# Xinglab/abPOA

Measured on AMD Instinct MI355X. Metric: read-sets/sec (consensus bit-exact) + DP Gcells/sec (roofline.dp_gcells_per_s), higher is better.
Workload: dtype int16

## Files before the change

### abpoa_amd/csrc/engine_options.cpp

```cpp
#include "engine_options.h"
#include <atomic>
#include <cstdlib>
#include <cstring>
#include <mutex>
#include <string>

namespace abpoa_hip {
namespace {

struct Row { const char *name, *help; };
const Row kTable[] = {
    {"ABPOA_GPU_DEVICES", "P  device ordinals abpoa_hip_msa_batch spreads its batches over: all | 0,1,... (default: the device of abpoa_hip_init)"},
    {"ABPOA_GPU_BATCHES_PER_DEVICE", "P  batches dealt per device queue [2]"},
    {"ABPOA_HIP_STRICT", "P  1: a call that would hand any read-set to the host driver fails with ABPOA_HIP_ESTRICT"},
    {"ABPOA_HIP_VERBOSE", "P  per-pass timings, residency and fallback reasons on stderr"},
    {"ABPOA_HIP_HOSTGRAPH", "T  1: the host driver for every job"},
    {"ABPOA_HIP_NO_DEVICE_STRAND", "T  1: -s jobs on the host driver"},
    {"ABPOA_HIP_NO_DEVICE_LOCAL", "T  1: local-mode jobs on the host driver"},
    {"ABPOA_HIP_NO_DEVICE_GENERAL", "T  1: general-kernel jobs on the host driver"},
    {"ABPOA_HIP_DEVICE_GENERAL", "T  1: the general kernel for every device-resident job"},
    {"ABPOA_HIP_LOCKSTEP", "T  1: one launch per phase and round also where the all-rounds kernel would run"},
    {"ABPOA_HIP_NODIR", "T  1: score-record arenas instead of direction words"},
    {"ABPOA_HIP_DIR_WIDE", "T  1 / 0: direction words for wide-band alignments always / never (default: by residency and memory)"},
    {"ABPOA_HIP_NOFAST", "T  1: no fast row loops (general kernel)"},
    {"ABPOA_HIP_NOWIDE", "T  1: no wide row loop"},
    {"ABPOA_HIP_NOXL", "T  1: no long-read form of the wide row loop"},
    {"ABPOA_HIP_TEAM", "T  1 | 2 | 4 wavefronts per wide-band alignment"},
    {"ABPOA_HIP_LOCAL_TEAM", "T  1 / 0: the four-wavefront local row loop always / never"},
    {"ABPOA_HIP_WIDE_LO", "T  smallest band half-width that takes the wide loop [40]"},
    {"ABPOA_HIP_RING_ROWS", "T  depth of the wide loop's score ring (4 | 8 | 16)"},
    {"ABPOA_HIP_EXTRA_ROUTE_MIN", "T  ragged sets with fewer extra columns keep the narrow loop"},
    {"ABPOA_HIP_NO_RAGGED_SPLIT", "T  1: read-sets with ragged read ends stay in the batch of the uniform ones (no all-rounds kernel for such a job)"},
    {"ABPOA_HIP_RAGGED_CONCURRENT", "T  1: the ragged batch of a mixed job runs on a second queue of the device beside the uniform batch (measured: see LOG.md)"},
    {"ABPOA_HIP_PASS_SETS", "T  read-sets per pass of the device-resident driver"},
    {"ABPOA_HIP_FIRST_PASS", "T  start the node-slot ladder at pass 1 / 2 / 3 (profiling runs of one step)"},
    {"ABPOA_HIP_NO_PASS_HINT", "T  1: always start the ladder at 3x"},
    {"ABPOA_HIP_GROUPS", "T  read-set groups of the host driver"},
    {"ABPOA_HIP_ARENA_PCT", "T  arena estimate in percent (overflow-retry tests)"},
    {"ABPOA_HIP_BT_BYTES", "T  LDS window of the tail kernel in bytes"},
    {"ABPOA_HIP_BT_WC", "T  columns per row of the tail's column-slice windows"},
    {"ABPOA_HIP_ORDER_LDS", "T  0: the row-order walk with global tables"},
    {"ABPOA_HIP_ORDER_CAP", "T  node capacity of the row-order walk's LDS tables"},
    {"ABPOA_HIP_DBG", "D  bit mask handed to the kernels (DevBatch.dbg: 64 no fast loops, 128 keep counters, 1024 one wavefront per backtrack, 2048 the compiler's tight loop, ...)"},
    {"ABPOA_HIP_DEVSYNC", "D  1: compare device graph / row order / MSA with the host's after every read"},
    {"ABPOA_HIP_DEVICE_AUDIT", "D  1: every pool of a device queue must sit on that queue's device"},
    {"ABPOA_HIP_CIGAR_DIGEST", "D  1: fold every graph cigar into a per-set digest on the device"},
    {"ABPOA_HIP_DIRTRACE", "D  1: keep direction words and scores (word-level tests)"},
    {"ABPOA_HIP_IMBAL", "D  1: per-round mean / slowest alignment"},
    {"ABPOA_HIP_WIDE_COUNTERS", "D  path census of the wide loop (diagnostic build)"},
    {"ABPOA_HIP_ROW_CENSUS", "D  row census of the narrow loop (diagnostic build)"},
    {"ABPOA_HIP_ORDER_PROF", "D  in-kernel clock of the row-order walk (diagnostic build)"},
};
constexpr int N = (int)(sizeof(kTable) / sizeof(kTable[0]));

struct Snap { bool set[N]; std::string val[N]; };
std::mutex g_mu;
bool g_over_on[N]; std::string g_over[N];
std::atomic<const Snap *> g_snap{nullptr};

int find(const char *name) { for (int i = 0; i < N; ++i) if (strcmp(kTable[i].name, name) == 0) return i; return -1; }

}

void refresh_options() {
    std::lock_guard<std::mutex> lk(g_mu);
    Snap s;
    for (int i = 0; i < N; ++i) {
        const char *e = g_over_on[i] ? g_over[i].c_str() : getenv(kTable[i].name);
        s.set[i] = e != nullptr; s.val[i] = e ? e : "";
    }
    const Snap *cur = g_snap.load(std::memory_order_acquire);
    bool same = cur != nullptr;
    for (int i = 0; same && i < N; ++i) same = cur->set[i] == s.set[i] && cur->val[i] == s.val[i];
    if (!same) g_snap.store(new Snap(s), std::memory_order_release);
}

// ... 22 lines not shown
```

### abpoa_amd/csrc/rows_fast.h

```cpp
#pragma once
#include "dp_common.h"
#include "dir_plane.h"
#include "rows_tight_asm.h"
#include "wide_closed_forms.h"

namespace abpoa_hip {

template <typename T, int GAP> struct FastFmt { static constexpr int CW = GAP == 0 ? 2 : (GAP == 1 ? 4 : 8); };
template <typename T, int GAP> struct DirFmt {
    static constexpr int DB = GAP == 1 ? 2 : 4;
    static constexpr int UPV2 = Width<T>::PN * DB / 16;
    __device__ __host__ static constexpr int units(int nv) { return (nv * UPV2 + 1) >> 1; }
};
template <int GAP> __device__ __forceinline__ unsigned dir_word(unsigned kf, unsigned u1, unsigned u2, unsigned d1, unsigned d2) {
    static_assert(DIRA_DF1_SH - DIRA_UE1_SH == 3 && DIRC_UE2_SH - DIRC_UE1_SH == 3 && DIRC_DF2_SH - DIRC_DF1_SH == 3 && DIRC_DF1_SH - DIRC_UE1_SH == 8, "field layout of dir_plane.h");
    if (GAP == 1) return (((d1 << 3) | u1) << DIRA_UE1_SH) | kf;
    return (((((d2 << 3) | d1) << 8) | ((u2 << 3) | u1)) << DIRC_UE1_SH) | kf;
}
template <int GAP> __device__ __forceinline__ unsigned dir_pack(unsigned kM, unsigned kE1, unsigned kE2, unsigned u1, unsigned u2, unsigned d1, unsigned d2) {
    return dir_word<GAP>(GAP == 1 ? (kE1 << DIRA_KE1_SH) | kM : (((kE2 << 4) | kE1) << DIRC_KE1_SH) | kM, u1, u2, d1, d2);
}
__device__ __forceinline__ unsigned umin_(unsigned a, unsigned b) { return a < b ? a : b; }
template <typename T> __device__ __forceinline__ unsigned dir_literal(int Hm1, int Fm1, int F, int oe, int e) {
    return (int)(T)(Hm1 - oe) == F ? (unsigned)DIR_LIT_OPEN : ((int)(T)(Fm1 - e) == F ? (unsigned)DIR_LIT_EXT : (unsigned)DIR_LIT_NEITHER);
// ... 100 lines not shown
    typedef __attribute__((address_space(3))) int lds_int_t;
    const int vslot = (int)(unsigned)(size_t)(lds_int_t *)fr + 4 * ((threadIdx.x & 63 & (RR - 1)) * (NPW * RCS) + 2);
    auto ring_at = [&](int slot_addr, int col_idx) __attribute__((always_inline)) { return (const int *)(lds_int_t *)(size_t)(unsigned)(slot_addr + 4 * col_idx); };
    int *s_mx = (int *)(lds_raw + (WPLAN ? b.lds.w_mx_off : b.lds.mx_off));
    auto qat = [&](int j) __attribute__((always_inline)) -> int {
        if constexpr (WPLAN) return ((int)s_query[j >> 1] >> ((j & 1) * 4)) & 15; else return (int)s_query[j];
    };
    const int infw = I16 ? (int)(((unsigned)inf & 0xffffu) | ((unsigned)inf << 16)) : inf;
    const int qlen_sn = qlen / PN;
    auto wr = [](int x) __attribute__((always_inline)) { return (int)(T)x; };

    const int idist = inj_dist<PN>(l);
    const int inj1 = idist >= 0 ? inf - idist * e1 : INT_MIN, inj2 = idist >= 0 ? inf - idist * e2 : INT_MIN;
    const int le1 = lane * e1, le2 = lane * e2;
    const int cf1 = oe1 - e1 + le1, cf2 = oe2 - e2 + le2;
    const long long lo_ll = (long long)(I16 ? INT16_MIN : INT32_MIN) + imax(oe1, oe2) + (long long)PN * imax(e1, e2);
    const int fast_lo = (int)lo_ll;
    const int kconst = I16 ? argmax_key16_const(PN, l, vvl) : 0;
    const int ktie = argmax_tie32(PN, l, vvl);

    { GLOBAL_AS const int32_t *g_mat = vgpr_ptr(b.mat); for (int i = tid; i < m * m1; i += NT) { const int bb = i / m1, qc = i - bb * m1; s_mx[i] = qc < m ? g_mat[bb * m + qc] : 0; } }
    for (int i = tid; i < RR * NPW * RCS; i += NT) { const int pl = (i / RCS) % NPW; fr[i] = (I16 && pl == 0) ? infw : ((EPACK && pl == 1) ? 0 : inf); }
    if (NW > 1 && tid < 16) xch[tid] = make_int4(INT_MIN, INT_MIN, I16 ? 0 : INT_MIN, 0);
    WG_SYNC();
    auto ring_put = [&](int slot, int x, int H, int E1, int E2) __attribute__((always_inline)) {
        int *q = fr + slot * (NPW * RCS) + 2 + x;
        if (I16) { q[0] = (int)(((unsigned)H & 0xffffu) | ((unsigned)E1 << 16)); if (GAP == 2) q[RCS] = E2; }
        else { q[0] = H; if (GAP != 0) q[RCS] = E1; if (GAP == 2) q[2 * RCS] = E2; }
    };

    const bool extend = sgpr(b.align_mode == ABPOA_HIP_EXTEND_MODE ? 1 : 0) != 0;
    int ex_best = inf, ex_i = 0, ex_j = 0, ex_rem = 0; bool zstop = false;
    const bool asm_tight_on = sgpr(!(b.dbg & 2048) && RC == 128 && b.align_mode != ABPOA_HIP_EXTEND_MODE ? 1 : 0) != 0;
    int cur = 0, n_vec_lane = 0;
    const int cap_pn = (int)(d.plane_cap / PN > 0x7fffffffLL ? 0x7fffffffLL : d.plane_cap / PN);
    const int cap_turbo = cap_pn - (DIR ? dir_units(NV) + NV * CWR : NV * CW);
    const int remain_end = __builtin_amdgcn_readfirstlane(io.row_remain[gn - 1]);
    int vg_geo = 0, vg_mi = 0, vg_off = 0;
    int vg_vm = 0, rowmax = 0;
    {
        const int r = __builtin_amdgcn_readfirstlane(io.row_remain[0]) - remain_end - 1;
        const int dp_end0 = imin(qlen, imax(0, qlen - r) + w);
        const int end_sn0 = dp_end0 / PN, W0 = (end_sn0 + 1) * PN;
        if ((long long)W0 * CWR > d.plane_cap) { status = ABPOA_HIP_STATUS_OVERFLOW; cursor_out = 0; n_cells_out = 0; rows_done_out = 0; return; }
        const bool ring0 = W0 <= RC && !EPACK;
        T *H = io.planes;
        for (int i = tid; i < W0; i += NT) {
            int h, x1 = inf, x2 = inf, f1 = inf, f2 = inf;
            if (GAP == 0) h = wr(-e1 * i);
            else if (GAP == 1) { const int g = wr(-o1 - e1 * i); h = i == 0 ? 0 : g; x1 = i == 0 ? wr(-oe1) : inf; f1 = i == 0 ? inf : g; }
            else {
                const int g1 = wr(-o1 - e1 * i), g2 = wr(-o2 - e2 * i);
                h = i == 0 ? 0 : imax(g1, g2); x1 = i == 0 ? wr(-oe1) : inf; x2 = i == 0 ? wr(-oe2) : inf; f1 = i == 0 ? inf : g1; f2 = i == 0 ? inf : g2;
            }
            T *cellp = H + (long long)i * CWR;
            if constexpr (CPK) { cellp[0] = (T)h; cellp[1] = (T)(i == 0 ? (int)((unsigned)(h - x1) | ((unsigned)(h - x2) << 16)) : -1); }
            else if constexpr (CSP) { cellp[0] = (T)h; cellp[PL_E1] = (T)x1; if (GAP == 2) { cellp[PL_E2] = (T)x2; cellp[3] = (T)0; } }
            else if constexpr (GAP == 0) { cellp[0] = (T)h; cellp[1] = (T)0; }
            else {
                cellp[0] = (T)h; cellp[PL_E1] = (T)x1; cellp[PL_F1] = (T)f1;
                if (GAP == 2) { cellp[PL_E2] = (T)x2; cellp[PL_F2] = (T)f2; }
            }
            if (ring0) ring_put(0, i, h, x1, x2);
        }
        cur = (end_sn0 + 1) * CWR;
        if (lane == 0) { vg_geo = (end_sn0 << 12) | (ring0 ? GEO_RING : 0); vg_mi = 0; vg_off = DIR ? cur : 0; }
// ... 12 lines not shown
    auto load_b = [&](const MetaA &a) __attribute__((always_inline)) {
        MetaB q; const int np = a.pe - a.ps;
#pragma unroll
        for (int k = 0; k < NPM; ++k) q.p[k] = io.pred_row[a.ps + imin(k, imax(np - 1, 0))];
        return q;
    };
    MetaA a1 = load_a(0); MetaB b1 = load_b(a1); MetaA a2 = load_a(64);
    int tv_r1 = 0, tv_r2 = 0;
    int tv_meta = 0, tv_rterm = 0, tv_ps = 0, tv_p0 = 0, tv_p1 = 0, tv_p2 = 0, tv_p3 = 0;
    int tv_p4 = 0, tv_p5 = 0, tv_p6 = 0, tv_p7 = 0;
    int tv_tb = 0;
    auto switch_tile = [&](int t0) __attribute__((always_inline)) {
        const int myrow = t0 + lane, np = a1.pe - a1.ps;
        bool fastrow = np >= 1 && np <= 4 && myrow < gn - 1 && myrow >= 1;
#pragma unroll
        for (int k = 0; k < 4; ++k) { const int dk = myrow - b1.p[k]; fastrow = fastrow && dk >= 1 && dk < RR; }
        tv_meta = (a1.base & 0xff) | (imin(np, 255) << 8) | (fastrow ? (1 << 16) : 0);
        if (!WPLAN) {
            tv_meta |= ((fastrow && np <= 2 && RC <= 128) ? (1 << 17) : 0) | ((fastrow && np >= 3 && RC <= 128) ? (1 << 18) : 0);
            bool row8 = np >= 5 && np <= 8 && myrow < gn - 1 && myrow >= 1 && RC <= 128;
#pragma unroll
            for (int k = 0; k < NPM; ++k) { const int dk = myrow - b1.p[k]; row8 = row8 && dk >= 1 && dk < RR; }
            tv_meta |= row8 ? (1 << 20) : 0;
        }
        {
            bool widerow = np >= 1 && np <= 8 && myrow < gn - 1 && myrow >= 1;
#pragma unroll
            for (int k = 0; k < NPM; ++k) { const int dk = myrow - b1.p[k]; widerow = widerow && dk >= 1 && dk < ((WIDEB || !WPLAN) ? 64 : RR); }
            tv_meta |= widerow ? (1 << 19) : 0;
        }
        if constexpr (DIR) {
            const bool sp = a1.sd >= RR;
            if (sp) { tv_meta |= 1 << 21; if (tv_meta & (1 << 17)) tv_meta = (tv_meta & ~(1 << 17)) | (1 << 22); }
        }
        tv_tb = ((myrow - b1.p[0]) & 0xff) | (((myrow - b1.p[1]) & 0xff) << 8) | (((a1.base & 0xff) * m1 * 4) << 16);
        tv_rterm = qlen - (a1.rem - remain_end - 1); tv_ps = a1.ps;
        tv_r1 = imin(gn, tv_rterm) - w; tv_r2 = tv_rterm + w;
        tv_p0 = b1.p[0]; tv_p1 = b1.p[1]; tv_p2 = b1.p[2]; tv_p3 = b1.p[3];
        tv_p4 = b1.p[4]; tv_p5 = b1.p[5]; tv_p6 = b1.p[6]; tv_p7 = b1.p[7];
        a1 = a2; b1 = load_b(a1); a2 = load_a(t0 + 128);
    };
    int qc_beg_sn = -1, qoff0 = 0, qoff1 = 0;
    auto geo_of = [&](int p, int row, int &geo, int &mi, int &off) __attribute__((always_inline)) {
        if (row - p < 64) { const int sl = p & 63; geo = __builtin_amdgcn_readlane(vg_geo, sl); mi = __builtin_amdgcn_readlane(vg_mi, sl); off = __builtin_amdgcn_readlane(vg_off, sl); }
        else {
            geo = __builtin_amdgcn_readfirstlane(gld_i32(io.g_bsn + p) | (gld_i32(io.g_esn + p) << 12)); mi = __builtin_amdgcn_readfirstlane(gld_i32(io.row_max_i + p));
            off = __builtin_amdgcn_readfirstlane((int)(uint32_t)(gld_i64(io.g_coff + p) / PN));
        }
    };
    int beg_sn = 0, end_sn = 0, off_pn = 0, max_pe = 0, rterm = 0, base = 0, np = 0;
    bool to_ring = false;
    unsigned am_key = 0; int am_val = INT_MIN, am_v = 0, am_isend = 0; bool am_any = false;

    auto set_band = [&](auto pin, int mn_mi, int mx_mi, int min_pb) __attribute__((always_inline)) {
        auto S = [](int x) __attribute__((always_inline)) { if constexpr (decltype(pin)::value) return sgpr(x); else return x; };
        const int left = S(imin(gn, mn_mi + 1)), right = S(decltype(pin)::value ? mx_mi + 1 : imax(0, mx_mi + 1));
        const int lo = S(imin(left, rterm) - w), hi = S(imax(right, rterm) + w);
        const int beg = S(imax(0, lo)), end = S(imin(qlen, hi));
        beg_sn = imax((int)((unsigned)beg / PN), min_pb); end_sn = (int)((unsigned)end / PN);
    };
    auto refresh_qc = [&]() __attribute__((always_inline)) {
        if (beg_sn != qc_beg_sn) {
            qc_beg_sn = beg_sn;
            const int c0 = beg_sn * PN + lane, c1 = c0 + 64;
            qoff0 = (c0 >= 1 && c0 <= qlen) ? qat(c0 - 1) : m; qoff1 = (c1 >= 1 && c1 <= qlen) ? qat(c1 - 1) : m;
        }
// ... 932 lines not shown
                            }
                        }
                    }
                    if (lane == 0) { bcast[0] = rc; bcast[1] = beg_sn; bcast[2] = end_sn; bcast[3] = off_pn; bcast[4] = mi; bcast[5] = to_ring ? 1 : 0; bcast[6] = cur; bcast[7] = rowmax; }
                }
                lds_barrier();
                rc = __builtin_amdgcn_readfirstlane(bcast[0]); beg_sn = __builtin_amdgcn_readfirstlane(bcast[1]); end_sn = __builtin_amdgcn_readfirstlane(bcast[2]);
                off_pn = __builtin_amdgcn_readfirstlane(bcast[3]); mi = __builtin_amdgcn_readfirstlane(bcast[4]); to_ring = __builtin_amdgcn_readfirstlane(bcast[5]) != 0;
                cur = __builtin_amdgcn_readfirstlane(bcast[6]); rowmax = __builtin_amdgcn_readfirstlane(bcast[7]);
                if (rc == 2) { status = ABPOA_HIP_STATUS_OVERFLOW; break; }
                commit_row(ti, to_ring);
                lds_barrier();
                ++row;
                continue;
            }
            int ok_ = 1;
            if constexpr (!WPLAN && GAP != 0) if (__builtin_expect(two_chunk_streak, 0)) {
                const int ti_ = row & 63, meta_ = __builtin_amdgcn_readlane(tv_meta, ti_);
                if constexpr (DIR) row_spill = (meta_ >> 21) & 1;
                if ((meta_ >> 19) & 1) {
                    CENSUS_T0()
                    last_done = row;
                    rterm = __builtin_amdgcn_readlane(tv_rterm, ti_); base = meta_ & 0xff; np = (meta_ >> 8) & 0xff;
                    const int nch_ = ilp_band(row, ti_);
                    if (nch_ == -2) { status = ABPOA_HIP_STATUS_OVERFLOW; break; }
                    if (nch_ == 2 && ilp_chunks(std::integral_constant<int, 2>{}, nch_, row, ti_) == 1) { commit_row(ti_, true); CENSUS(3) ++row; continue; }
                }
                two_chunk_streak = 0;
            }
            bool cxx_tight = true;
#if !defined(ABPOA_HIP_ABLATE) && !defined(ABPOA_HIP_PROFILE) && (!defined(ABPOA_HIP_ROW_CENSUS) || defined(ABPOA_HIP_ASM_CENSUS)) && !defined(ABPOA_HIP_NO_ASM_TIGHT)
            if constexpr (!WPLAN && I16 && GAP == 1 && DIR) {
                if (asm_tight_on && cur + NV * (r_hi - row) <= cap_turbo) {
                    int code, sM, sTB, sRT, sR2, sP0, sM0, sG0, sSL0, sA, sB, sESN, sBSN, sPB0, sPE0, sNV1, sC0, sP1, sM1, sG1, sSL1, sPB1, sPE1, sP2, sSL2, sPB2, sPE2, sP3, sSL3, sPB3, sPE3;
                    long long inb, amok, msk;
#ifdef ABPOA_HIP_ASM_CENSUS
                    const int asm_row0 = row; const long long asm_t0 = (long long)__builtin_amdgcn_s_memtime();
#endif
                    int infw_v = infw, inf_v = inf; asm("" : "+v"(infw_v), "+v"(inf_v));
                    const int mxb = (int)(unsigned)(size_t)(lds_int_t *)s_mx, qb = (int)(unsigned)(size_t)(lds_int_t *)(const void *)s_query;
                    asm volatile(TIGHT_ASM_I16_AFFINE_DIR
                        : [row] "+s"(row), [cur] "+s"(cur), [qcb] "+s"(qc_beg_sn), [code] "=&s"(code), [geo] "+v"(vg_geo), [mi] "+v"(vg_mi), [off] "+v"(vg_off), [qoff0] "+v"(qoff0),
                          [qoff1] "+v"(qoff1), [sM] "=&s"(sM), [sTB] "=&s"(sTB), [sRT] "=&s"(sRT), [sR2] "=&s"(sR2), [sP0] "=&s"(sP0), [sM0] "=&s"(sM0), [sG0] "=&s"(sG0), [sSL0] "=&s"(sSL0), [sA] "=&s"(sA),
                          [sB] "=&s"(sB), [sESN] "=&s"(sESN), [sBSN] "=&s"(sBSN), [sPB0] "=&s"(sPB0), [sPE0] "=&s"(sPE0), [sNV1] "=&s"(sNV1), [sC0] "=&s"(sC0), [sP1] "=&s"(sP1),
                          [sM1] "=&s"(sM1), [sG1] "=&s"(sG1), [sSL1] "=&s"(sSL1), [sPB1] "=&s"(sPB1), [sPE1] "=&s"(sPE1), [sP2] "=&s"(sP2), [sSL2] "=&s"(sSL2), [sPB2] "=&s"(sPB2),
                          [sPE2] "=&s"(sPE2), [sP3] "=&s"(sP3), [sSL3] "=&s"(sSL3), [sPB3] "=&s"(sPB3), [sPE3] "=&s"(sPE3), [inb] "=&s"(inb), [amok] "=&s"(amok), [msk] "=&s"(msk)
                        : [lane] "v"(lane), [tvmeta] "v"(tv_meta), [tvtb] "v"(tv_tb), [tvr1] "v"(tv_r1), [tvr2] "v"(tv_r2), [tvp2] "v"(tv_p2), [tvp3] "v"(tv_p3), [vslot] "v"(vslot), [le1] "v"(le1), [cf1] "v"(cf1), [inj1] "v"(inj1), [kN] "v"(kN),
                          [kE] "v"(kE), [vvl] "v"(vvl), [vl] "v"(l), [infwv] "v"(infw_v), [infv] "v"(inf_v), [c1] "s"(1 - w), [c2] "s"(1 + w), [qlen] "s"(qlen), [rc] "s"(RC), [mxb] "s"(mxb), [fastlo] "s"(fast_lo),
                          [e1] "s"(e1), [oe1] "s"(oe1), [infk] "s"((int)((((unsigned)(inf + 32768)) << 16) | 0xffffu)), [planes] "s"(io.planes), [rhi] "s"(r_hi), [qb] "s"(qb), [m] "s"(m), [perm] "s"(0x05040100)
                        : "v92", "v93", "v94", "v95", "v96", "v97", "v98", "v99", "v100", "v101", "v102", "v103", "v104", "v105", "v106", "v107", "v108", "v109", "v110", "v111", "v112", "v113", "v114", "v115", "v116", "v117", "v118", "v119",
                          "v120", "v121", "v122", "v123", "v124", "v125", "v126", "v127", "vcc", "scc", "m0", "memory");
                    ok_ = code == 1 ? 0 : (code == 2 ? -1 : 1);
                    cxx_tight = false;
#ifdef ABPOA_HIP_ASM_CENSUS
                    fseg[0] += ((long long)(row - asm_row0) << 40) + ((long long)__builtin_amdgcn_s_memtime() - asm_t0);
#endif
                }
            }
#endif
            if constexpr (!WPLAN) if (cxx_tight) for (;;) {
                const int ti_ = row & 63;
                const int meta_ = __builtin_amdgcn_readlane(tv_meta, ti_);
                if (!__builtin_expect((meta_ >> 17) & 1, 1)) break;
                if constexpr (DIR) row_spill = (meta_ >> 21) & 1;
                CENSUS_T0()
                rterm = __builtin_amdgcn_readlane(tv_rterm, ti_);
                base = meta_ & 0xff; np = (meta_ >> 8) & 0xff;
                ok_ = np == 1 ? turbo_body(std::integral_constant<int, 1>{}, std::false_type{}, row, ti_) : turbo_body(std::integral_constant<int, 2>{}, std::false_type{}, row, ti_);
                if (__builtin_expect(ok_ != 1, 0)) break;
                commit_row(ti_, true);
                CENSUS(np == 1 ? 0 : 1)
                if (++row >= r_hi || zstop) break;
            }
            last_done = row - 1;
            if (row >= r_hi || zstop) break;
            const int ti = row & 63;
            last_done = row;
            CENSUS_T0()
            const int meta = __builtin_amdgcn_readlane(tv_meta, ti);
            rterm = __builtin_amdgcn_readlane(tv_rterm, ti);
// ... 134 lines not shown
```

### abpoa_amd/csrc/rows_tight_asm.h

```cpp
#pragma once
#define TA_SDWA0 " dst_sel:DWORD dst_unused:UNUSED_PAD src0_sel:WORD_0 src1_sel:DWORD\n\t"
#define TA_SDWA_S1W0 " dst_sel:DWORD dst_unused:UNUSED_PAD src0_sel:DWORD src1_sel:WORD_0\n\t"
#define TA_SDWA_S1W1 " dst_sel:DWORD dst_unused:UNUSED_PAD src0_sel:DWORD src1_sel:WORD_1\n\t"
#define TA_SDWA_S0W1 " dst_sel:DWORD dst_unused:UNUSED_PAD src0_sel:WORD_1 src1_sel:DWORD\n\t"
#define TA_DPP(CTRL) " " CTRL " bank_mask:0xf\n\t"
#define vQA "v104"
#define vCOL "v105"
#define vX "v106"
#define vQ "v107"
#define vR0 "v108"
#define vR1 "v109"
#define vR01 "v[108:109]"
#define vKC "v110"
#define vH "v111"
#define vHSE "v112"
#define vAK "v113"
#define vS1 "v114"
#define vG "v115"
#define vF "v115"
#define vQD "v116"
#define vRO "v117"
#define vHO "v118"
#define vT2A "v119"
#define vEN "v120"
// ... 130 lines not shown
    S("v_lshl_or_b32 " vWD ", " vSH ", 14, " vWD "\n\t")                                                     \
    "global_store_short " vRO ", " vWD ", %[planes]\n\t"                                                     \
    "v_cndmask_b32_e64 " vHE ", %[infwv], " vHE ", %[inb]\n\t"                                                   \
    "ds_write2st64_b32 " vQD ", " vHE ", %[infwv] offset1:1\n\t"                                             \
    "v_readlane_b32 %[sA], " vAK ", 63\n\t"                                                                  \
    "s_bitset1_b32 %[sB], 24\n\t"                                                                            \
    "v_writelane_b32 %[geo], %[sB], m0\n\t"     "v_writelane_b32 %[off], %[cur], m0\n\t"                     \
    "s_and_b32 %[sM0], %[sA], 63\n\t"           "s_add_i32 %[sM0], %[sM0], %[sC0]\n\t"                       \
    "s_cmp_gt_u32 %[sA], %[infk]\n\t"           "s_cselect_b32 %[sA], %[sM0], -1\n\t"       \
    "v_writelane_b32 %[mi], %[sA], m0\n\t"                                                                   \
    "s_add_i32 %[cur], %[cur], %[sNV1]\n\t"     "s_add_i32 %[cur], %[cur], 1\n\t"                            \
    "s_add_i32 %[row], %[row], 1\n\t"           "s_cmp_lt_i32 %[row], %[rhi]\n\t"     "s_cbranch_scc1 L_row_%=\n\t"

#define TA_IF4_YES(x) x
#define TA_IF4_NO(x) ""
#define TA_FOLD(LANE, SL, PB, PE)                                                                            \
    "v_readlane_b32 %[sM1], %[mi], " LANE "\n\t"  "v_readlane_b32 %[sG1], %[geo], " LANE "\n\t"  "v_readlane_b32 " SL ", %[vslot], " LANE "\n\t" \
    "s_min_i32 %[sA], %[sA], %[sM1]\n\t"          "s_max_i32 %[sB], %[sB], %[sM1]\n\t"           "s_and_b32 %[sG0], %[sG0], %[sG1]\n\t" \
    "s_and_b32 " PB ", %[sG1], 0xfff\n\t"         "s_bfe_u32 " PE ", %[sG1], 0xc000c\n\t"
#define TA_READK(X, PAIR, SL, PB, PE)                                                                        \
    "s_lshl_b32 %[sA], " PB ", 4\n\t"             "v_subrev_u32 " X ", %[sA], " vCOL "\n\t"                  \
    "v_add_u32 " vT ", -1, " X "\n\t"             "v_med3_i32 " vT ", " vT ", -2, %[rc]\n\t"                 \
    "v_lshl_add_u32 " vT ", " vT ", 2, " SL "\n\t"  "ds_read2_b32 " PAIR ", " vT " offset1:1\n\t"            \
    "s_sub_i32 " PE ", " PE ", " PB "\n\t"        "s_lshl_b32 " PE ", " PE ", 4\n\t"             "s_add_i32 " PE ", " PE ", 16\n\t"
#define TA_MERGE(KIDX, W0, W1, X, PE)                                                                        \
    "v_max_i32_sdwa " vT ", " vMV ", sext(" W0 ")" TA_SDWA_S1W0                                              \
    "v_cmp_lt_i32 vcc, " vMV ", " vT "\n\t"                                                                  \
    "s_add_i32 %[sA], " PE ", 16\n\t"             "v_cmp_gt_u32_e64 %[msk], %[sA], " X "\n\t"    "s_and_b64 vcc, vcc, %[msk]\n\t" \
    "v_cndmask_b32_e64 " vKM ", " vKM ", " KIDX ", vcc\n\t"   "v_cndmask_b32_e64 " vMV ", " vMV ", " vT ", %[msk]\n\t" \
    "v_max_i32_sdwa " vT ", " vE1 ", sext(" W1 ")" TA_SDWA_S1W1                                              \
    "v_cmp_lt_i32 vcc, " vE1 ", " vT "\n\t"                                                                  \
    "v_cmp_gt_u32_e64 %[msk], " PE ", " X "\n\t"  "s_and_b64 vcc, vcc, %[msk]\n\t"                           \
    "v_cndmask_b32_e64 " vKE ", " vKE ", " KIDX ", vcc\n\t"   "v_cndmask_b32_e64 " vE1 ", " vE1 ", " vT ", %[msk]\n\t"
#define TA_MULTI_POST(IF4, S)                                                                                \
    TA_RINGCHK                                                                                               \
    TA_MASKS                                                                                                 \
    "v_mov_b32 " vKM ", 1\n\t"                    "v_mov_b32 " vKE ", 1\n\t"                                 \
    "s_waitcnt lgkmcnt(0)\n\t"                                                                               \
    "v_bfe_i32 " vMV ", " vR0 ", 0, 16\n\t"       "v_ashrrev_i32 " vE1 ", 16, " vR1 "\n\t"                   \
    TA_MERGE("2", vB0, vB1, vX1, "%[sPE1]")                                                                  \
    TA_MERGE("3", vC0, vC1, vX2, "%[sPE2]")                                                                  \
    IF4(TA_MERGE("4", vD0, vD1, vX3, "%[sPE3]"))                                                             \
    "v_add_u32 " vH ", " vMV ", " vQ "\n\t"                                                                  \
    "v_min_i32 " vT ", " vH ", " vE1 "\n\t"                                                                  \
    "v_cmp_gt_i32 vcc, %[fastlo], " vT "\n\t"     "s_and_b64 %[msk], %[inb], vcc\n\t"   "s_cbranch_scc1 L_x2_%=\n\t"  \
    "v_max_i32 " vHSE ", " vH ", " vE1 "\n\t"                                                                \
    TA_SCAN                                                                                                  \
    S(TA_SLOW_A)                                                                                             \
    TA_HEF("v_subrev_u32 " vEN ", %[e1], " vE1 "\n\t", S)                                                    \
    "v_cmp_eq_u32 vcc, " vH ", " vHO "\n\t"       "v_cndmask_b32 " vKF ", 0, " vKM ", vcc\n\t"               \
    "v_lshl_or_b32 " vKF ", " vKE ", 4, " vKF "\n\t"                                                         \
    TA_TAIL(S)                                                                                               \
    "s_branch L_end_%=\n\t"
#define TA_MULTI(IF4, LBL)                                                                                   \
    "s_mov_b32 %[sA], %[sM0]\n\t"                 "s_mov_b32 %[sB], %[sM0]\n\t"                              \
    "s_and_b32 %[sPB0], %[sG0], 0xfff\n\t"        "s_bfe_u32 %[sPE0], %[sG0], 0xc000c\n\t"                   \
    TA_FOLD("%[sP1]", "%[sSL1]", "%[sPB1]", "%[sPE1]")                                                       \
    TA_FOLD("%[sP2]", "%[sSL2]", "%[sPB2]", "%[sPE2]")                                                       \
    IF4(TA_FOLD("%[sP3]", "%[sSL3]", "%[sPB3]", "%[sPE3]"))                                                  \
    "s_add_i32 %[sA], %[sA], %[c1]\n\t"               "s_add_i32 %[sB], %[sB], %[c2]\n\t"                            \
    TA_BAND_BEG                                                                                              \
    "s_min_u32 %[sESN], %[sPB0], %[sPB1]\n\t"     "s_min_u32 %[sESN], %[sESN], %[sPB2]\n\t"   IF4("s_min_u32 %[sESN], %[sESN], %[sPB3]\n\t") \
    "s_max_u32 %[sBSN], %[sA], %[sESN]\n\t"                                                                  \
    TA_QCACHE(LBL)                                                                                           \
    TA_READS                                                                                                 \
    "s_max_u32 %[sPE0], %[sPE0], %[sPE1]\n\t"     "s_max_u32 %[sPE0], %[sPE0], %[sPE2]\n\t" IF4("s_max_u32 %[sPE0], %[sPE0], %[sPE3]\n\t") \
    TA_READK(vX1, vB01, "%[sSL1]", "%[sPB1]", "%[sPE1]")                                                     \
    TA_READK(vX2, vC01, "%[sSL2]", "%[sPB2]", "%[sPE2]")                                                     \
    IF4(TA_READK(vX3, vD01, "%[sSL3]", "%[sPB3]", "%[sPE3]"))                                                \
    TA_BAND_END                                                                                              \
    TA_CHECKS("L_s" LBL)                                                                                     \
    TA_MULTI_POST(IF4, TA_S_NO)                                                                              \
    TA_SLOW_ENTRY("L_s" LBL)                                                                                 \
    TA_MULTI_POST(IF4, TA_S_YES)

#define TA_ONE_POST(S)                                                                                       \
    TA_RINGCHK                                                                                               \
    TA_MASKS                                                                                                 \
    "s_waitcnt lgkmcnt(0)\n\t"                                                                               \
    "v_add_u32_sdwa " vH ", sext(" vR0 "), " vQ TA_SDWA0                                                     \
    "v_min_i32_sdwa " vT ", " vH ", sext(" vR1 ")" TA_SDWA_S1W1                                              \
    "v_cmp_gt_i32 vcc, %[fastlo], " vT "\n\t"   "s_and_b64 %[msk], %[inb], vcc\n\t"   "s_cbranch_scc1 L_x2_%=\n\t"  \
    "v_max_i32_sdwa " vHSE ", " vH ", sext(" vR1 ")" TA_SDWA_S1W1                                            \
    TA_SCAN                                                                                                  \
    S(TA_SLOW_A)                                                                                             \
    TA_HEF("v_sub_u32_sdwa " vEN ", sext(" vR1 "), %[e1]" TA_SDWA_S0W1, S)                                   \
    "v_cmp_eq_u32 vcc, " vH ", " vHO "\n\t"     "v_cndmask_b32_e64 " vKF ", 16, 17, vcc\n\t"                 \
    TA_TAIL(S)                                                                                               \
    "s_branch L_end_%=\n\t"
#define TA_TWO_POST(S)                                                                                       \
    TA_RINGCHK                                                                                               \
    TA_MASKS                                                                                                 \
    "s_waitcnt lgkmcnt(0)\n\t"                                                                               \
    "v_bfe_i32 " vMV ", " vR0 ", 0, 16\n\t"     "v_ashrrev_i32 " vE1 ", 16, " vR1 "\n\t"                     \
    "v_max_i32_sdwa " vT ", " vMV ", sext(" vB0 ")" TA_SDWA_S1W0                                             \
    "v_cmp_gt_u32 vcc, %[sP1], " vX1 "\n\t"     "v_cndmask_b32 " vMV2 ", " vMV ", " vT ", vcc\n\t"           \
    "v_max_i32_sdwa " vT ", " vE1 ", sext(" vB1 ")" TA_SDWA_S1W1                                             \
    "v_cmp_gt_u32 vcc, %[sM1], " vX1 "\n\t"     "v_cndmask_b32 " vE12 ", " vE1 ", " vT ", vcc\n\t"           \
    "v_add_u32 " vH ", " vMV2 ", " vQ "\n\t"                                                                 \
    "v_min_i32 " vT ", " vH ", " vE12 "\n\t"                                                                 \
    "v_cmp_gt_i32 vcc, %[fastlo], " vT "\n\t"   "s_and_b64 %[msk], %[inb], vcc\n\t"   "s_cbranch_scc1 L_x2_%=\n\t"  \
    "v_max_i32 " vHSE ", " vH ", " vE12 "\n\t"                                                               \
    TA_SCAN                                                                                                  \
    S(TA_SLOW_A)                                                                                             \
    TA_HEF("v_subrev_u32 " vEN ", %[e1], " vE12 "\n\t", S)                                                   \
    "v_cmp_ne_u32 vcc, " vMV2 ", " vMV "\n\t"   "v_cndmask_b32_e64 " vKF ", 1, 2, vcc\n\t"                   \
    "v_cmp_eq_u32 vcc, " vH ", " vHO "\n\t"     "v_cndmask_b32 " vKF ", 0, " vKF ", vcc\n\t"                 \
// ... 28 lines not shown
    TA_QCACHE("1")                                                                                           \
    TA_READS                                                                                                 \
    TA_BAND_END                                                                                              \
    "s_bfe_u32 %[sPE0], %[sG0], 0xc000c\n\t"                                                                 \
    TA_CHECKS("L_s1")                                                                                        \
    TA_ONE_POST(TA_S_NO)                                                                                     \
    TA_SLOW_ENTRY("L_s1")                                                                                    \
    TA_ONE_POST(TA_S_YES)                                                                                    \
                                                                      \
    TA_ALIGN "L_two_%=:\n\t"                                                                                          \
    "s_bfe_u32 %[sA], %[sTB], 0x80008\n\t"      "s_sub_i32 %[sP1], %[row], %[sA]\n\t"                        \
    "v_readlane_b32 %[sM1], %[mi], %[sP1]\n\t"  "v_readlane_b32 %[sG1], %[geo], %[sP1]\n\t"   "v_readlane_b32 %[sSL1], %[vslot], %[sP1]\n\t" \
    "s_min_i32 %[sA], %[sM0], %[sM1]\n\t"       "s_max_i32 %[sB], %[sM0], %[sM1]\n\t"                        \
    "s_add_i32 %[sA], %[sA], %[c1]\n\t"             "s_add_i32 %[sB], %[sB], %[c2]\n\t"                              \
    TA_BAND_BEG                                                                                              \
    "s_and_b32 %[sPB0], %[sG0], 0xfff\n\t"      "s_and_b32 %[sPB1], %[sG1], 0xfff\n\t"                       \
    "s_min_u32 %[sESN], %[sPB0], %[sPB1]\n\t"   "s_max_u32 %[sBSN], %[sA], %[sESN]\n\t"                      \
    TA_QCACHE("2")                                                                                           \
    TA_READS                                                                                                 \
    "s_lshl_b32 %[sA], %[sPB1], 4\n\t"          "v_subrev_u32 " vX1 ", %[sA], " vCOL "\n\t"                  \
    "v_add_u32 " vX ", -1, " vX1 "\n\t"         "v_med3_i32 " vX ", " vX ", -2, %[rc]\n\t"                   \
    "v_lshl_add_u32 " vX ", " vX ", 2, %[sSL1]\n\t"   "ds_read2_b32 " vB01 ", " vX " offset1:1\n\t"           \
    TA_BAND_END                                                                                              \
    "s_bfe_u32 %[sPE0], %[sG0], 0xc000c\n\t"    "s_bfe_u32 %[sPE1], %[sG1], 0xc000c\n\t"                     \
    "s_sub_i32 %[sM1], %[sPE1], %[sPB1]\n\t"    "s_lshl_b32 %[sM1], %[sM1], 4\n\t"                           \
    "s_add_i32 %[sM1], %[sM1], 16\n\t"          "s_add_i32 %[sP1], %[sM1], 16\n\t"                           \
    "s_max_u32 %[sPE0], %[sPE0], %[sPE1]\n\t"   "s_and_b32 %[sG0], %[sG0], %[sG1]\n\t"                       \
    TA_CHECKS("L_s2")                                                                                        \
    TA_TWO_POST(TA_S_NO)                                                                                     \
    TA_SLOW_ENTRY("L_s2")                                                                                    \
    TA_TWO_POST(TA_S_YES)                                                                                    \
                                                             \
    TA_ALIGN "L_n17_%=:\n\t"                                                                                          \
    "s_bitcmp1_b32 %[sM], 18\n\t"               "s_cbranch_scc0 L_x0_%=\n\t"                                 \
    "s_bitcmp1_b32 %[sM], 21\n\t"               "s_cbranch_scc1 L_x0_%=\n\t"                                 \
    "v_readlane_b32 %[sP2], %[tvp2], %[row]\n\t"  "v_readlane_b32 %[sP3], %[tvp3], %[row]\n\t"               \
    "s_bfe_u32 %[sA], %[sTB], 0x80008\n\t"      "s_sub_i32 %[sP1], %[row], %[sA]\n\t"                        \
    "s_bitcmp1_b32 %[sM], 10\n\t"               "s_cbranch_scc1 L_four_%=\n\t"                               \
    TA_MULTI(TA_IF4_NO, "3")                                                                                 \
    TA_ALIGN "L_four_%=:\n\t"                                                                                         \
    TA_MULTI(TA_IF4_YES, "4")                                                                                \
                                                                           \
    TA_REFRESH("1")                                                                                          \
    TA_REFRESH("2")                                                                                          \
    TA_REFRESH("3")                                                                                          \
    TA_REFRESH("4")                                                                                          \
    "L_dec_%=:\n\t"                                                                                          \
    "s_waitcnt lgkmcnt(0)\n\t"                   \
    "s_mov_b32 %[code], 2\n\t"                                                                               \
    "s_cmp_gt_u32 %[sNV1], 3\n\t"               "s_cbranch_scc1 L_end_%=\n\t"                                \
    "s_cmp_gt_i32 %[sBSN], %[sPE0]\n\t"         "s_cbranch_scc1 L_end_%=\n\t"                                \
    "s_bitcmp0_b32 %[sG0], 24\n\t"              "s_cbranch_scc1 L_end_%=\n\t"                                \
    "s_mov_b32 %[code], 1\n\t"                  "s_branch L_end_%=\n\t"                                      \
    "L_x0_%=:\n\t"  "s_mov_b32 %[code], 0\n\t"  "s_branch L_end_%=\n\t"                                      \
    "L_x2_%=:\n\t"  "s_mov_b32 %[code], 2\n\t"                                                               \
    "L_end_%=:\n\t"
```

Before: 18450.

## Handle rows with five to eight predecessors inside the assembly tight loop

Adds an eight-predecessor path to the hand-written tight row loop. Rows whose predecessor count is 5-8 get metadata bit 23 and are folded, read and merged in assembly instead of leaving the loop for the slower general path. More SGPR operands and VGPRs are used, and a debug bit (4096) turns the path off. The extra register pressure and code size could cost occupancy or add instruction-cache misses.

After: 18640 (median of 6 runs). 1.01x the previous value.

```diff
diff --git a/abpoa_amd/csrc/engine_options.cpp b/abpoa_amd/csrc/engine_options.cpp
--- a/abpoa_amd/csrc/engine_options.cpp
+++ b/abpoa_amd/csrc/engine_options.cpp
@@ -41,7 +41,7 @@
     {"ABPOA_HIP_BT_WC", "T  columns per row of the tail's column-slice windows"},
     {"ABPOA_HIP_ORDER_LDS", "T  0: the row-order walk with global tables"},
     {"ABPOA_HIP_ORDER_CAP", "T  node capacity of the row-order walk's LDS tables"},
-    {"ABPOA_HIP_DBG", "D  bit mask handed to the kernels (DevBatch.dbg: 64 no fast loops, 128 keep counters, 1024 one wavefront per backtrack, 2048 the compiler's tight loop, ...)"},
+    {"ABPOA_HIP_DBG", "D  bit mask handed to the kernels (DevBatch.dbg: 64 no fast loops, 128 keep counters, 1024 one wavefront per backtrack, 2048 the compiler's tight loop, 4096 rows with 5-8 predecessors stay out of the assembly loop, ...)"},
     {"ABPOA_HIP_DEVSYNC", "D  1: compare device graph / row order / MSA with the host's after every read"},
     {"ABPOA_HIP_DEVICE_AUDIT", "D  1: every pool of a device queue must sit on that queue's device"},
     {"ABPOA_HIP_CIGAR_DIGEST", "D  1: fold every graph cigar into a per-set digest on the device"},
diff --git a/abpoa_amd/csrc/rows_fast.h b/abpoa_amd/csrc/rows_fast.h
--- a/abpoa_amd/csrc/rows_fast.h
+++ b/abpoa_amd/csrc/rows_fast.h
@@ -156,6 +156,7 @@
     const bool extend = sgpr(b.align_mode == ABPOA_HIP_EXTEND_MODE ? 1 : 0) != 0;
     int ex_best = inf, ex_i = 0, ex_j = 0, ex_rem = 0; bool zstop = false;
     const bool asm_tight_on = sgpr(!(b.dbg & 2048) && RC == 128 && b.align_mode != ABPOA_HIP_EXTEND_MODE ? 1 : 0) != 0;
+    const bool asm_row8_on = sgpr(!(b.dbg & 4096) ? 1 : 0) != 0;
     int cur = 0, n_vec_lane = 0;
     const int cap_pn = (int)(d.plane_cap / PN > 0x7fffffffLL ? 0x7fffffffLL : d.plane_cap / PN);
     const int cap_turbo = cap_pn - (DIR ? dir_units(NV) + NV * CWR : NV * CW);
@@ -234,6 +235,7 @@
         if constexpr (DIR) {
             const bool sp = a1.sd >= RR;
             if (sp) { tv_meta |= 1 << 21; if (tv_meta & (1 << 17)) tv_meta = (tv_meta & ~(1 << 17)) | (1 << 22); }
+            else if (!WPLAN && (tv_meta & (1 << 20)) && asm_row8_on) tv_meta |= 1 << 23;
         }
         tv_tb = ((myrow - b1.p[0]) & 0xff) | (((myrow - b1.p[1]) & 0xff) << 8) | (((a1.base & 0xff) * m1 * 4) << 16);
         tv_rterm = qlen - (a1.rem - remain_end - 1); tv_ps = a1.ps;
@@ -1232,7 +1234,7 @@
 #if !defined(ABPOA_HIP_ABLATE) && !defined(ABPOA_HIP_PROFILE) && (!defined(ABPOA_HIP_ROW_CENSUS) || defined(ABPOA_HIP_ASM_CENSUS)) && !defined(ABPOA_HIP_NO_ASM_TIGHT)
             if constexpr (!WPLAN && I16 && GAP == 1 && DIR) {
                 if (asm_tight_on && cur + NV * (r_hi - row) <= cap_turbo) {
-                    int code, sM, sTB, sRT, sR2, sP0, sM0, sG0, sSL0, sA, sB, sESN, sBSN, sPB0, sPE0, sNV1, sC0, sP1, sM1, sG1, sSL1, sPB1, sPE1, sP2, sSL2, sPB2, sPE2, sP3, sSL3, sPB3, sPE3;
+                    int code, sM, sTB, sRT, sR2, sP0, sM0, sG0, sSL0, sA, sB, sESN, sBSN, sPB0, sPE0, sNV1, sC0, sP1, sM1, sG1, sSL1, sPB1, sPE1, sP2, sSL2, sPB2, sPE2, sP3, sSL3, sPB3, sPE3, sSL4, sG4, sSL5, sG5, sSL6, sG6, sSL7, sG7;
                     long long inb, amok, msk;
 #ifdef ABPOA_HIP_ASM_CENSUS
                     const int asm_row0 = row; const long long asm_t0 = (long long)__builtin_amdgcn_s_memtime();
@@ -1244,8 +1246,9 @@
                           [qoff1] "+v"(qoff1), [sM] "=&s"(sM), [sTB] "=&s"(sTB), [sRT] "=&s"(sRT), [sR2] "=&s"(sR2), [sP0] "=&s"(sP0), [sM0] "=&s"(sM0), [sG0] "=&s"(sG0), [sSL0] "=&s"(sSL0), [sA] "=&s"(sA),
                           [sB] "=&s"(sB), [sESN] "=&s"(sESN), [sBSN] "=&s"(sBSN), [sPB0] "=&s"(sPB0), [sPE0] "=&s"(sPE0), [sNV1] "=&s"(sNV1), [sC0] "=&s"(sC0), [sP1] "=&s"(sP1),
                           [sM1] "=&s"(sM1), [sG1] "=&s"(sG1), [sSL1] "=&s"(sSL1), [sPB1] "=&s"(sPB1), [sPE1] "=&s"(sPE1), [sP2] "=&s"(sP2), [sSL2] "=&s"(sSL2), [sPB2] "=&s"(sPB2),
-                          [sPE2] "=&s"(sPE2), [sP3] "=&s"(sP3), [sSL3] "=&s"(sSL3), [sPB3] "=&s"(sPB3), [sPE3] "=&s"(sPE3), [inb] "=&s"(inb), [amok] "=&s"(amok), [msk] "=&s"(msk)
-                        : [lane] "v"(lane), [tvmeta] "v"(tv_meta), [tvtb] "v"(tv_tb), [tvr1] "v"(tv_r1), [tvr2] "v"(tv_r2), [tvp2] "v"(tv_p2), [tvp3] "v"(tv_p3), [vslot] "v"(vslot), [le1] "v"(le1), [cf1] "v"(cf1), [inj1] "v"(inj1), [kN] "v"(kN),
+                          [sPE2] "=&s"(sPE2), [sP3] "=&s"(sP3), [sSL3] "=&s"(sSL3), [sPB3] "=&s"(sPB3), [sPE3] "=&s"(sPE3), [sSL4] "=&s"(sSL4), [sG4] "=&s"(sG4), [sSL5] "=&s"(sSL5), [sG5] "=&s"(sG5),
+                          [sSL6] "=&s"(sSL6), [sG6] "=&s"(sG6), [sSL7] "=&s"(sSL7), [sG7] "=&s"(sG7), [inb] "=&s"(inb), [amok] "=&s"(amok), [msk] "=&s"(msk)
+                        : [lane] "v"(lane), [tvmeta] "v"(tv_meta), [tvtb] "v"(tv_tb), [tvr1] "v"(tv_r1), [tvr2] "v"(tv_r2), [tvp2] "v"(tv_p2), [tvp3] "v"(tv_p3), [tvp4] "v"(tv_p4), [tvp5] "v"(tv_p5), [tvp6] "v"(tv_p6), [tvp7] "v"(tv_p7), [vslot] "v"(vslot), [le1] "v"(le1), [cf1] "v"(cf1), [inj1] "v"(inj1), [kN] "v"(kN),
                           [kE] "v"(kE), [vvl] "v"(vvl), [vl] "v"(l), [infwv] "v"(infw_v), [infv] "v"(inf_v), [c1] "s"(1 - w), [c2] "s"(1 + w), [qlen] "s"(qlen), [rc] "s"(RC), [mxb] "s"(mxb), [fastlo] "s"(fast_lo),
                           [e1] "s"(e1), [oe1] "s"(oe1), [infk] "s"((int)((((unsigned)(inf + 32768)) << 16) | 0xffffu)), [planes] "s"(io.planes), [rhi] "s"(r_hi), [qb] "s"(qb), [m] "s"(m), [perm] "s"(0x05040100)
                         : "v92", "v93", "v94", "v95", "v96", "v97", "v98", "v99", "v100", "v101", "v102", "v103", "v104", "v105", "v106", "v107", "v108", "v109", "v110", "v111", "v112", "v113", "v114", "v115", "v116", "v117", "v118", "v119",
diff --git a/abpoa_amd/csrc/rows_tight_asm.h b/abpoa_amd/csrc/rows_tight_asm.h
--- a/abpoa_amd/csrc/rows_tight_asm.h
+++ b/abpoa_amd/csrc/rows_tight_asm.h
@@ -186,15 +186,15 @@
     "v_cmp_lt_i32 vcc, " vE1 ", " vT "\n\t"                                                                  \
     "v_cmp_gt_u32_e64 %[msk], " PE ", " X "\n\t"  "s_and_b64 vcc, vcc, %[msk]\n\t"                           \
     "v_cndmask_b32_e64 " vKE ", " vKE ", " KIDX ", vcc\n\t"   "v_cndmask_b32_e64 " vE1 ", " vE1 ", " vT ", %[msk]\n\t"
-#define TA_MULTI_POST(IF4, S)                                                                                \
+#define TA_MULTI_POST_A                                                                                      \
     TA_RINGCHK                                                                                               \
     TA_MASKS                                                                                                 \
     "v_mov_b32 " vKM ", 1\n\t"                    "v_mov_b32 " vKE ", 1\n\t"                                 \
     "s_waitcnt lgkmcnt(0)\n\t"                                                                               \
     "v_bfe_i32 " vMV ", " vR0 ", 0, 16\n\t"       "v_ashrrev_i32 " vE1 ", 16, " vR1 "\n\t"                   \
     TA_MERGE("2", vB0, vB1, vX1, "%[sPE1]")                                                                  \
-    TA_MERGE("3", vC0, vC1, vX2, "%[sPE2]")                                                                  \
-    IF4(TA_MERGE("4", vD0, vD1, vX3, "%[sPE3]"))                                                             \
+    TA_MERGE("3", vC0, vC1, vX2, "%[sPE2]")
+#define TA_MULTI_POST_B(S)                                                                                   \
     "v_add_u32 " vH ", " vMV ", " vQ "\n\t"                                                                  \
     "v_min_i32 " vT ", " vH ", " vE1 "\n\t"                                                                  \
     "v_cmp_gt_i32 vcc, %[fastlo], " vT "\n\t"     "s_and_b64 %[msk], %[inb], vcc\n\t"   "s_cbranch_scc1 L_x2_%=\n\t"  \
@@ -206,6 +206,10 @@
     "v_lshl_or_b32 " vKF ", " vKE ", 4, " vKF "\n\t"                                                         \
     TA_TAIL(S)                                                                                               \
     "s_branch L_end_%=\n\t"
+#define TA_MULTI_POST(IF4, S)                                                                                \
+    TA_MULTI_POST_A                                                                                          \
+    IF4(TA_MERGE("4", vD0, vD1, vX3, "%[sPE3]"))                                                             \
+    TA_MULTI_POST_B(S)
 #define TA_MULTI(IF4, LBL)                                                                                   \
     "s_mov_b32 %[sA], %[sM0]\n\t"                 "s_mov_b32 %[sB], %[sM0]\n\t"                              \
     "s_and_b32 %[sPB0], %[sG0], 0xfff\n\t"        "s_bfe_u32 %[sPE0], %[sG0], 0xc000c\n\t"                   \
@@ -227,6 +231,78 @@
     TA_MULTI_POST(IF4, TA_S_NO)                                                                              \
     TA_SLOW_ENTRY("L_s" LBL)                                                                                 \
     TA_MULTI_POST(IF4, TA_S_YES)
+
+#define vX4 "v111"
+#define vX5 "v120"
+#define vX6 "v121"
+#define vX7 "v122"
+#define vN40 "v112"
+#define vN41 "v113"
+#define vN401 "v[112:113]"
+#define vN50 "v114"
+#define vN51 "v115"
+#define vN501 "v[114:115]"
+#define vN60 "v116"
+#define vN61 "v117"
+#define vN601 "v[116:117]"
+#define vN70 "v118"
+#define vN71 "v119"
+#define vN701 "v[118:119]"
+#define TA_FOLD8(LANE, SL, G)                                                                                \
+    "v_readlane_b32 %[sM1], %[mi], " LANE "\n\t"  "v_readlane_b32 " G ", %[geo], " LANE "\n\t"   "v_readlane_b32 " SL ", %[vslot], " LANE "\n\t" \
+    "s_min_i32 %[sA], %[sA], %[sM1]\n\t"          "s_max_i32 %[sB], %[sB], %[sM1]\n\t"           "s_and_b32 %[sG0], %[sG0], " G "\n\t" \
+    "s_and_b32 %[sG1], " G ", 0xfff\n\t"          "s_min_u32 %[sESN], %[sESN], %[sG1]\n\t"                   \
+    "s_bfe_u32 %[sG1], " G ", 0xc000c\n\t"        "s_max_u32 %[sPE0], %[sPE0], %[sG1]\n\t"
+#define TA_READK8(X, PAIR, SL, G)                                                                            \
+    "s_and_b32 %[sM1], " G ", 0xfff\n\t"          "s_bfe_u32 " G ", " G ", 0xc000c\n\t"                      \
+    "s_lshl_b32 %[sA], %[sM1], 4\n\t"             "v_subrev_u32 " X ", %[sA], " vCOL "\n\t"                  \
+    "v_add_u32 " vT ", -1, " X "\n\t"             "v_med3_i32 " vT ", " vT ", -2, %[rc]\n\t"                 \
+    "v_lshl_add_u32 " vT ", " vT ", 2, " SL "\n\t"  "ds_read2_b32 " PAIR ", " vT " offset1:1\n\t"            \
+    "s_sub_i32 " G ", " G ", %[sM1]\n\t"          "s_lshl_b32 " G ", " G ", 4\n\t"             "s_add_i32 " G ", " G ", 16\n\t"
+#define TA_MULTI8_POST(S, L)                                                                                 \
+    TA_MULTI_POST_A                                                                                          \
+    TA_MERGE("4", vD0, vD1, vX3, "%[sPE3]")                                                                  \
+    TA_MERGE("5", vN40, vN41, vX4, "%[sG4]")                                                                 \
+    "s_cmp_lt_u32 %[sP3], 6\n\t"                  "s_cbranch_scc1 L_mg" L "_%=\n\t"                          \
+    TA_MERGE("6", vN50, vN51, vX5, "%[sG5]")                                                                 \
+    "s_cmp_lt_u32 %[sP3], 7\n\t"                  "s_cbranch_scc1 L_mg" L "_%=\n\t"                          \
+    TA_MERGE("7", vN60, vN61, vX6, "%[sG6]")                                                                 \
+    "s_cmp_lt_u32 %[sP3], 8\n\t"                  "s_cbranch_scc1 L_mg" L "_%=\n\t"                          \
+    TA_MERGE("8", vN70, vN71, vX7, "%[sG7]")                                                                 \
+    "L_mg" L "_%=:\n\t"                                                                                      \
+    TA_MULTI_POST_B(S)
+#define TA_MULTI8(LBL)                                                                                       \
+    "s_mov_b32 %[sA], %[sM0]\n\t"                 "s_mov_b32 %[sB], %[sM0]\n\t"                              \
+    "s_and_b32 %[sPB0], %[sG0], 0xfff\n\t"        "s_bfe_u32 %[sPE0], %[sG0], 0xc000c\n\t"                   \
+    TA_FOLD("%[sP1]", "%[sSL1]", "%[sPB1]", "%[sPE1]")                                                       \
+    "v_readlane_b32 %[sP1], %[tvp6], %[row]\n\t"                                                             \
+    TA_FOLD("%[sP2]", "%[sSL2]", "%[sPB2]", "%[sPE2]")                                                       \
+    "v_readlane_b32 %[sP2], %[tvp7], %[row]\n\t"                                                             \
+    TA_FOLD("%[sP3]", "%[sSL3]", "%[sPB3]", "%[sPE3]")                                                       \
+    "s_min_u32 %[sESN], %[sPB0], %[sPB1]\n\t"     "s_min_u32 %[sESN], %[sESN], %[sPB2]\n\t"   "s_min_u32 %[sESN], %[sESN], %[sPB3]\n\t" \
+    "s_max_u32 %[sPE0], %[sPE0], %[sPE1]\n\t"     "s_max_u32 %[sPE0], %[sPE0], %[sPE2]\n\t"   "s_max_u32 %[sPE0], %[sPE0], %[sPE3]\n\t" \
+    TA_FOLD8("%[sC0]", "%[sSL4]", "%[sG4]")                                                                  \
+    TA_FOLD8("%[sNV1]", "%[sSL5]", "%[sG5]")                                                                 \
+    TA_FOLD8("%[sP1]", "%[sSL6]", "%[sG6]")                                                                  \
+    TA_FOLD8("%[sP2]", "%[sSL7]", "%[sG7]")                                                                  \
+    "s_bfe_u32 %[sP3], %[sM], 0x80008\n\t"                \
+    "s_add_i32 %[sA], %[sA], %[c1]\n\t"           "s_add_i32 %[sB], %[sB], %[c2]\n\t"                        \
+    TA_BAND_BEG                                                                                              \
+    "s_max_u32 %[sBSN], %[sA], %[sESN]\n\t"                                                                  \
+    TA_QCACHE(LBL)                                                                                           \
+    TA_READS                                                                                                 \
+    TA_READK(vX1, vB01, "%[sSL1]", "%[sPB1]", "%[sPE1]")                                                     \
+    TA_READK(vX2, vC01, "%[sSL2]", "%[sPB2]", "%[sPE2]")                                                     \
+    TA_READK(vX3, vD01, "%[sSL3]", "%[sPB3]", "%[sPE3]")                                                     \
+    TA_READK8(vX4, vN401, "%[sSL4]", "%[sG4]")                                                               \
+    TA_READK8(vX5, vN501, "%[sSL5]", "%[sG5]")                                                               \
+    TA_READK8(vX6, vN601, "%[sSL6]", "%[sG6]")                                                               \
+    TA_READK8(vX7, vN701, "%[sSL7]", "%[sG7]")                                                               \
+    TA_BAND_END                                                                                              \
+    TA_CHECKS("L_s" LBL)                                                                                     \
+    TA_MULTI8_POST(TA_S_NO, LBL "f")                                                                         \
+    TA_SLOW_ENTRY("L_s" LBL)                                                                                 \
+    TA_MULTI8_POST(TA_S_YES, LBL "s")
 
 #define TA_ONE_POST(S)                                                                                       \
     TA_RINGCHK                                                                                               \
@@ -321,7 +397,7 @@
     TA_TWO_POST(TA_S_YES)                                                                                    \
                                                              \
     TA_ALIGN "L_n17_%=:\n\t"                                                                                          \
-    "s_bitcmp1_b32 %[sM], 18\n\t"               "s_cbranch_scc0 L_x0_%=\n\t"                                 \
+    "s_bitcmp1_b32 %[sM], 18\n\t"               "s_cbranch_scc0 L_n18_%=\n\t"                                \
     "s_bitcmp1_b32 %[sM], 21\n\t"               "s_cbranch_scc1 L_x0_%=\n\t"                                 \
     "v_readlane_b32 %[sP2], %[tvp2], %[row]\n\t"  "v_readlane_b32 %[sP3], %[tvp3], %[row]\n\t"               \
     "s_bfe_u32 %[sA], %[sTB], 0x80008\n\t"      "s_sub_i32 %[sP1], %[row], %[sA]\n\t"                        \
@@ -329,11 +405,19 @@
     TA_MULTI(TA_IF4_NO, "3")                                                                                 \
     TA_ALIGN "L_four_%=:\n\t"                                                                                         \
     TA_MULTI(TA_IF4_YES, "4")                                                                                \
+                                                            \
+    TA_ALIGN "L_n18_%=:\n\t"                                                                                 \
+    "s_bitcmp1_b32 %[sM], 23\n\t"               "s_cbranch_scc0 L_x0_%=\n\t"                                 \
+    "v_readlane_b32 %[sP2], %[tvp2], %[row]\n\t"  "v_readlane_b32 %[sP3], %[tvp3], %[row]\n\t"               \
+    "v_readlane_b32 %[sC0], %[tvp4], %[row]\n\t"  "v_readlane_b32 %[sNV1], %[tvp5], %[row]\n\t"              \
+    "s_bfe_u32 %[sA], %[sTB], 0x80008\n\t"      "s_sub_i32 %[sP1], %[row], %[sA]\n\t"                        \
+    TA_MULTI8("8")                                                                                           \
                                                                            \
     TA_REFRESH("1")                                                                                          \
     TA_REFRESH("2")                                                                                          \
     TA_REFRESH("3")                                                                                          \
     TA_REFRESH("4")                                                                                          \
+    TA_REFRESH("8")                                                                                          \
     "L_dec_%=:\n\t"                                                                                          \
     "s_waitcnt lgkmcnt(0)\n\t"                   \
     "s_mov_b32 %[code], 2\n\t"                                                                               \
```
